# ethanhe42/epipolar-transformers

Hardware: AMD Instinct MI355X
Metric: multi-view images/sec at H36M 4-view 256x256 bs=32 (pair-views/s, whole layer forward) (higher is better)
Workload: dtype f32 (split-fp16 MFMA, f32 accumulate); 1 GPU; configs[1]: epipolarposeR head, 4 views x 32 frames = 128 pairs/GPU, C=256, 64x64, K=64, z+BN+residual, eval; partition=frames, layout=NHWC (channels_last), pairs_per_gpu=128, variant=0, launch=kernel by kernel from Python

## Files before the change

epipolar_transformers_amd/_lib.py:

```python
from __future__ import annotations

import ctypes
import os

_PKG = os.path.dirname(os.path.abspath(__file__))
LIB_PATH = os.environ.get("EPIPOLAR_AMD_LIB") or os.path.join(_PKG, "lib", "libepipolar_amd.so")

ET_CAM_STRIDE = 27
ET_VARIANT_SAFE_REDUCE = 1
ET_VARIANT_NO_TAP_CACHE = 2
ET_VARIANT_PIXEL_INTERLEAVE = 4
ET_VARIANT_BATCH4 = 8
ET_VARIANT_OCC5 = 16
ET_VARIANT_OCC6 = 32
ET_VARIANT_BASELINE = 256
ET_VARIANT_PIPELINE = 512
ET_VARIANT_MULTI2 = 1024
ET_VARIANT_MULTI4 = 2048
ET_VARIANT_BWD_ATOMIC = 4096
ET_VARIANT_BWD_UNSORTED = 8192
ET_VARIANT_NO_TILE = 16384
ET_VARIANT_TILE_SPLIT = 32768
ET_VARIANT_TILE_CLASSIC = 65536
ET_VARIANT_WS_SETPRIO = 262144
ET_VARIANT_TILE_EXACT = 524288
ET_VARIANT_WS_BAND = 1048576
ET_VARIANT_BWD_SPLIT_IN_PLACE = 2097152
ET_ABI_VERSION = 13
ET_GENERAL_POOLING = 1
ET_GENERAL_PRIOR_MUL = 2
ET_GENERAL_COSINE = 4
ET_GENERAL_ATTENTION_MAX = 8
ET_GENERAL_SIM_PRIOR = 16


class EpipolarAmdError(RuntimeError):
    pass


class EtLayerDesc(ctypes.Structure):

    _fields_ = [
        ("N", ctypes.c_int32), ("C", ctypes.c_int32), ("H", ctypes.c_int32), ("W", ctypes.c_int32),
        ("K", ctypes.c_int32),
        ("xmin", ctypes.c_float), ("ymin", ctypes.c_float), ("xmax", ctypes.c_float), ("ymax", ctypes.c_float),
        ("eps", ctypes.c_float), ("downsample", ctypes.c_float),
        ("image_resize", ctypes.c_float), ("predict_resize", ctypes.c_float),
        ("correct_normalize", ctypes.c_int32), ("align_corners", ctypes.c_int32),
        ("softmax_scale", ctypes.c_float), ("softmax_enabled", ctypes.c_int32),
        ("src_grad_mask", ctypes.c_int32), ("variant", ctypes.c_int32),
    ]


_P = ctypes.c_void_p
_D = ctypes.POINTER(EtLayerDesc)
_SIGNATURES = {
    "et_abi_version": (ctypes.c_int, []),
    "et_last_error": (ctypes.c_char_p, []),
    "et_sample_locs": (ctypes.c_int, [_D, _P, _P, _P, _P, _P, _P]),
    "et_epipolar_forward": (ctypes.c_int, [_D, _P, _P, _P, _P, _P, _P, _P, _P, _P, _P, _P, _P]),
    "et_epipolar_forward_general": (ctypes.c_int, [_D] + [_P] * 8 + [ctypes.c_int32] * 3 + [_P] * 4),
    "et_epipolar_backward_general": (ctypes.c_int, [_D] + [_P] * 9 + [ctypes.c_int32] * 3 + [_P] * 5),
    "et_epipolar_forward_workspace_bytes": (ctypes.c_size_t, [_D]),
    "et_epipolar_forward_workspace_stats_offset": (ctypes.c_size_t, [_D]),
    "et_epipolar_forward_workspace_error_offset": (ctypes.c_size_t, [_D]),
    "et_epipolar_forward_tiled": (ctypes.c_int, [_D] + [_P] * 12 + [ctypes.c_size_t, _P]),
    "et_epipolar_forward_fused": (ctypes.c_int, [_D] + [_P] * 12 + [ctypes.c_int32, _P, ctypes.c_size_t, _P]),
    "et_epipolar_backward_tiled_workspace_bytes": (ctypes.c_size_t, [_D]),
    "et_epipolar_backward_tiled": (ctypes.c_int, [_D, _P, _P, _P, _P, _P, _P, _P, _P, _P, _P, ctypes.c_size_t, _P]),
    "et_epipolar_backward_tiled_attn": (ctypes.c_int, [_D, _P, _P, _P, _P, _P, _P, _P, _P, _P, _P, _P, ctypes.c_size_t, _P]),
    "et_epipolar_backward_workspace_bytes": (ctypes.c_size_t, [_D]),
    "et_epipolar_backward": (ctypes.c_int, [_D, _P, _P, _P, _P, _P, _P, _P, _P, _P, _P, ctypes.c_size_t, _P]),
    "et_residual_epilogue": (ctypes.c_int, [ctypes.c_int64, ctypes.c_int32, _P, _P, _P, _P, _P, _P, _P, _P]),
    "et_residual_gemm_packed_bytes": (ctypes.c_size_t, []),
    "et_residual_gemm_pack": (ctypes.c_int, [_P, _P, _P]),
    "et_residual_gemm": (ctypes.c_int, [ctypes.c_int64, ctypes.c_int32, _P, _P, _P, _P, _P, _P]),
    "et_z_batch_stats_workspace_bytes": (ctypes.c_size_t, [ctypes.c_int64]),
    "et_z_batch_stats": (ctypes.c_int, [ctypes.c_int64, ctypes.c_int32, _P, _P, _P, _P, _P, _P, _P, ctypes.c_size_t, _P]),
    "et_z_wgrad_workspace_bytes": (ctypes.c_size_t, [ctypes.c_int64]),
    "et_z_wgrad": (ctypes.c_int, [ctypes.c_int64, ctypes.c_int32, _P, _P, _P, _P, _P, ctypes.c_size_t, _P]),
    "et_z_backward_workspace_bytes": (ctypes.c_size_t, [ctypes.c_int64]),
    "et_z_backward": (ctypes.c_int, [ctypes.c_int64, ctypes.c_int32, _P, _P, _P, _P, _P, _P, ctypes.c_int32, _P, _P, _P, _P, _P,
                                     ctypes.c_size_t, _P]),
    "et_heatmap_peaks": (ctypes.c_int, [ctypes.c_int64, ctypes.c_int32, ctypes.c_int32, _P, ctypes.c_float, ctypes.c_float,
                                        ctypes.c_float, ctypes.c_int32, _P, _P, _P]),
    "et_nchw_to_nhwc": (ctypes.c_int, [ctypes.c_int32] * 4 + [_P, _P, _P]),
    "et_nhwc_to_nchw": (ctypes.c_int, [ctypes.c_int32] * 4 + [_P, _P, _P]),
    "et_debug_host_sample_setup": (ctypes.c_int, [_D, _P, _P, _P, _P, ctypes.c_int32, ctypes.c_int32, _P, _P, _P]),
    "et_debug_atomic_probe": (ctypes.c_int, [_P, ctypes.c_int64, ctypes.c_int32, ctypes.c_int32, _P]),
}

_lib = None


def exported_symbols():
    return sorted(_SIGNATURES)


def load():
    global _lib
    if _lib is not None:
        return _lib
    if not os.path.exists(LIB_PATH):
        raise EpipolarAmdError(
            "HIP library %s not found. Build it with `python -m epipolar_transformers_amd.build` "
            "(hipcc, gfx950). There is no CPU fallback for this path." % LIB_PATH)
    lib = ctypes.CDLL(LIB_PATH)
    for name, (res, args) in _SIGNATURES.items():
        fn = getattr(lib, name)
        fn.restype = res
# ... 13 lines not shown
```

epipolar_transformers_amd/csrc/et_tile_host.h:

```cpp
#pragma once
#include <algorithm>
namespace {
int tile_rows_per_pixel(const EtLayerDesc *d)
{
    const int longest = d->W > d->H ? d->W : d->H;
    return (d->K < longest) ? 4 * d->K : 4 * longest;
}
int tile_rows(const EtLayerDesc *d)
{
    if (tile_rows_per_pixel(d) > kTileRowsLarge) return kTileRowsHuge;
    return (d->W > 64 || d->H > 64) ? kTileRowsLarge : kTileRowsSmall;
}
int tile_rows_cap(const EtLayerDesc *d) { return (d->variant & ET_VARIANT_TILE_SPLIT) ? 64 : tile_rows(d); }

bool tile_eligible(const EtLayerDesc *d)
{
    if (d->C != 256 || d->K > 256) return false;
    const long long hw = (long long)d->H * d->W;
    if (hw > 16384) return false;
    return tile_rows_per_pixel(d) <= tile_rows_cap(d);
}

bool tile_ws_band(const EtLayerDesc *d)
{
    const int longest = d->W > d->H ? d->W : d->H;
    if ((d->variant & ET_VARIANT_TILE_CLASSIC) || !d->softmax_enabled || d->K > 64 || d->W < 2 || longest > kWsMaxSideBand)
        return false;
    return tile_rows(d) == kTileRowsLarge || ((d->variant & ET_VARIANT_WS_BAND) && tile_rows(d) == kTileRowsSmall);
}
bool tile_ws_two_pass(const EtLayerDesc *d)
{
    const int longest = d->W > d->H ? d->W : d->H;
    return !(d->variant & ET_VARIANT_TILE_CLASSIC) && d->softmax_enabled && d->K > 64 && d->K <= 128 && d->W >= 2 && longest <= kWsMaxSideTwoPass;
}
bool tile_ws_eligible(const EtLayerDesc *d)
{
    return (!(d->variant & ET_VARIANT_TILE_CLASSIC) && d->softmax_enabled && d->K <= 64 && d->W >= 2 &&
            tile_rows(d) == kTileRowsSmall) || tile_ws_band(d);
}
struct TileWorkspace {
    int *perm, *ovf_count, *err, *ovf_list, *stats;
    float *scales;
    float4 *segs, *band, *segs_pix;
};
constexpr size_t kTileWorkspaceHeaderWords = 64;
size_t tile_workspace_words(size_t tiles, size_t pairs, size_t hw)
{
    return kTileWorkspaceHeaderWords + tiles * kTilePix + 2 * tiles + 4 * pairs + 4 + 4 * tiles * kTilePix + 4 * tiles +
           4 * pairs * hw;
}
TileWorkspace carve_tile_workspace(void *workspace, size_t tiles, size_t pairs, size_t hw)
{
    TileWorkspace w;
    w.ovf_count = reinterpret_cast<int *>((reinterpret_cast<uintptr_t>(workspace) + 255) & ~(uintptr_t)255);
    w.err = w.ovf_count + 1;
    w.perm = w.ovf_count + kTileWorkspaceHeaderWords;
    w.ovf_list = w.perm + tiles * kTilePix;
    w.stats = w.ovf_list + tiles;
    w.scales = reinterpret_cast<float *>(w.stats + tiles);
    w.segs = reinterpret_cast<float4 *>((reinterpret_cast<uintptr_t>(w.scales + 4 * pairs) + 15) & ~(uintptr_t)15);
    w.band = w.segs + tiles * kTilePix;
    w.segs_pix = w.band + tiles;
    return w;
}

int launch_tile_order(const EtLayerDesc *desc, const float *xs, const float *ys, const float *cam, const float *feat_ref,
                      const float *feat_src, const TileWorkspace &w, int tiles_per_pair, bool header, float *scales,
                      bool ws_tables, float4 *clear, size_t clear_vec4, hipStream_t st, const char *who)
{
    const int HW = desc->H * desc->W;
    const int perm_stride = tiles_per_pair * kTilePix;
    int n2 = 64;
    while (n2 < HW) n2 <<= 1;
    const size_t lds_sort = order_uses_radix(n2) ? ((tile_order_lds_bytes(n2) + 15) & ~(size_t)15) + order_radix_extra_bytes(n2)
                                                 : tile_order_lds_bytes(n2);
    const int dev = current_device();
    ET_GRANT_LDS(tile_order_kernel, lds_sort, dev);
    unsigned long long *keys = reinterpret_cast<unsigned long long *>(w.segs);
    hipLaunchKernelGGL(tile_keys_kernel, dim3((unsigned)((HW + 255) / 256) * desc->N), dim3(256), 0, st, *desc, xs, ys, cam, perm_stride,
                       keys, w.segs_pix, header ? w.ovf_count : (int *)nullptr);
    const unsigned clear_blocks = clear ? (unsigned)std::min<size_t>(2048, (clear_vec4 + 8 * 1024 - 1) / (8 * 1024)) : 0u;
    hipLaunchKernelGGL(tile_order_kernel, dim3(desc->N + clear_blocks), dim3(1024), lds_sort, st, *desc, n2, perm_stride, keys,
                       w.segs_pix, w.perm, feat_ref, feat_src, scales, ws_tables ? w.segs : (float4 *)nullptr,
                       ws_tables ? w.band : (float4 *)nullptr, clear, clear_vec4);
    return check_launch(who);
}
}
```

epipolar_transformers_amd/csrc/kernels_forward_tile.inc:

```

typedef float f32x16 __attribute__((ext_vector_type(16)));

constexpr int kTilePix = 32;
constexpr int kTileRowsSmall = 256, kTileRowsLarge = 384, kTileRowsHuge = 512;
constexpr int kTileRowsWsLarge = 288, kWsMaxSideBand = 96, kWsMaxSideTwoPass = 128;

struct TileParams {
    FwdParams f;
    const int *perm;
    int tiles_per_pair;
    int hw_words;
    int *stats;
    int rows_cap;
    const int *tile_list;
    const int *tile_count;
    const float *scales;
};

__device__ __host__ constexpr int order_key_slot(int i) { return i + (i >> 4); }
constexpr size_t tile_order_lds_bytes(int n2) { return (size_t)order_key_slot(n2) * sizeof(unsigned long long); }
__device__ __forceinline__ unsigned long long order_key(unsigned k32, int j)
{
    return (unsigned long long)__double_as_longlong((double)(((unsigned long long)k32 << 14) | (unsigned)j));
}
constexpr unsigned long long kOrderPadKey = 0x42E0000000000000ull;
__device__ __forceinline__ int order_key_pixel(unsigned long long bits)
{
    return (int)((unsigned long long)__longlong_as_double((long long)bits) & 0x3FFFull);
}
template <int S>
__device__ __forceinline__ void order_sort_round(unsigned long long *s_key, int n2, int k, int jj_top)
{
    constexpr int R = 1 << S;
    const int jlow = jj_top >> (S - 1);
    for (int t = threadIdx.x; t < (n2 >> S); t += blockDim.x) {
        const int base = ((t & ~(jlow - 1)) << S) | (t & (jlow - 1));
        const unsigned long long flip = (base & k) == 0 ? 0ull : 0x8000000000000000ull;
        double v[R];
#pragma unroll
        for (int r = 0; r < R; ++r) v[r] = __longlong_as_double((long long)(s_key[order_key_slot(base + r * jlow)] ^ flip));
#pragma unroll
        for (int st = S - 1; st >= 0; --st)
#pragma unroll
            for (int r = 0; r < R; ++r)
                if (!(r & (1 << st))) {
                    const double a = v[r], b = v[r | (1 << st)];
                    double lo, hi;
                    asm("v_min_f64 %0, %1, %2" : "=v"(lo) : "v"(a), "v"(b));
                    asm("v_max_f64 %0, %1, %2" : "=v"(hi) : "v"(a), "v"(b));
                    v[r] = lo;
                    v[r | (1 << st)] = hi;
                }
#pragma unroll
        for (int r = 0; r < R; ++r) s_key[order_key_slot(base + r * jlow)] = (unsigned long long)__double_as_longlong(v[r]) ^ flip;
    }
    __syncthreads();
}

#ifndef ET_ORDER_RADIX
#define ET_ORDER_RADIX 0
#endif
constexpr int kOrderRadixMaxKeys = 4096, kOrderRadixMinKeys = 256;
__host__ __device__ constexpr bool order_uses_radix(int n2) { return ET_ORDER_RADIX != 0 && n2 >= kOrderRadixMinKeys && n2 <= kOrderRadixMaxKeys; }
constexpr size_t order_radix_extra_bytes(int n2) { return (size_t)n2 * 8 + (size_t)256 * (n2 >> 6) * 2 + 64; }

template <int PER>
__device__ __forceinline__ void order_radix_scan(unsigned short *s_cnt, unsigned *s_wtot)
{
    const int lane = threadIdx.x & 63, wave = threadIdx.x >> 6;
    unsigned v[PER];
    if constexpr (PER == 1) {
        v[0] = s_cnt[threadIdx.x];
    } else {
        const unsigned *src = reinterpret_cast<const unsigned *>(s_cnt) + threadIdx.x * (PER / 2);
#pragma unroll
        for (int i = 0; i < PER / 2; ++i) {
            const unsigned w = src[i];
            v[2 * i] = w & 0xFFFFu;
            v[2 * i + 1] = w >> 16;
        }
    }
    unsigned sum = 0;
#pragma unroll
    for (int i = 0; i < PER; ++i) {
        const unsigned c = v[i];
        v[i] = sum;
        sum += c;
    }
    unsigned incl = sum;
#pragma unroll
    for (int m = 1; m < kWave; m <<= 1) {
        const unsigned o = __shfl_up(incl, m);
        if (lane >= m) incl += o;
    }
    if (lane == kWave - 1) s_wtot[wave] = incl;
    __syncthreads();
    unsigned base = incl - sum;
    for (int w = 0; w < wave; ++w) base += s_wtot[w];
    if constexpr (PER == 1) {
        s_cnt[threadIdx.x] = (unsigned short)(base + v[0]);
    } else {
        unsigned *dst = reinterpret_cast<unsigned *>(s_cnt) + threadIdx.x * (PER / 2);
#pragma unroll
        for (int i = 0; i < PER / 2; ++i) dst[i] = ((base + v[2 * i]) & 0xFFFFu) | ((base + v[2 * i + 1]) << 16);
    }
}

__device__ __forceinline__ void order_radix_sort(unsigned long long *s_key, int n2, int HW)
{
    const int lane = threadIdx.x & 63, wave = threadIdx.x >> 6;
    const int G = n2 >> 6;
    unsigned long long *s_b = s_key + ((order_key_slot(n2) + 1) & ~1);
    unsigned short *s_cnt = reinterpret_cast<unsigned short *>(s_b + n2);
    unsigned *s_wtot = reinterpret_cast<unsigned *>(s_cnt + 256 * G);
    constexpr int kRounds = kOrderRadixMaxKeys / 64 / 16;
    const unsigned long long lt = (1ull << lane) - 1ull;
#pragma unroll 1
    for (int pass = 0; pass < 4; ++pass) {
        const bool fwd = (pass & 1) == 0;
        for (int i = threadIdx.x; i < 128 * G; i += blockDim.x) reinterpret_cast<unsigned *>(s_cnt)[i] = 0u;
        unsigned long long key[kRounds];
        int dgt[kRounds], rank[kRounds], cnt[kRounds];
#pragma unroll
        for (int r = 0; r < kRounds; ++r) {
            const int g = wave + 16 * r;
            dgt[r] = rank[r] = cnt[r] = 0;
            key[r] = 0ull;
            if (g < G) {
                const int i = g * kWave + lane;
                unsigned long long k = fwd ? s_key[order_key_slot(i)] : s_b[i];
                if (pass == 0) {
                    k = (i < HW) ? (unsigned long long)__longlong_as_double((long long)k) : ((0xFFFFFFFFull << 14) | (unsigned)i);
                }
                key[r] = k;
                const int d8 = (int)(k >> (14 + 8 * pass)) & 255;
                unsigned long long peers = ~0ull;
#pragma unroll
                for (int b = 0; b < 8; ++b) {
                    const bool bit = (d8 >> b) & 1;
                    const unsigned long long bal = __builtin_amdgcn_ballot_w64(bit);
                    peers &= bit ? bal : ~bal;
                }
                dgt[r] = d8;
                rank[r] = __popcll(peers & lt);
                cnt[r] = __popcll(peers);
            }
        }
        __syncthreads();
#pragma unroll
        for (int r = 0; r < kRounds; ++r) {
            const int g = wave + 16 * r;
            if (g < G && rank[r] == 0) s_cnt[dgt[r] * G + g] = (unsigned short)cnt[r];
        }
        __syncthreads();
        switch (G) {
        case 64: order_radix_scan<16>(s_cnt, s_wtot); break;
        case 32: order_radix_scan<8>(s_cnt, s_wtot); break;
        case 16: order_radix_scan<4>(s_cnt, s_wtot); break;
        case 8: order_radix_scan<2>(s_cnt, s_wtot); break;
        default: order_radix_scan<1>(s_cnt, s_wtot); break;
        }
        __syncthreads();
#pragma unroll
        for (int r = 0; r < kRounds; ++r) {
            const int g = wave + 16 * r;
            if (g < G) {
                const int pos = (int)s_cnt[dgt[r] * G + g] + rank[r];
                if (pass == 3) {
                    const int pix = (int)(key[r] & 0x3FFFull);
                    s_key[order_key_slot(pos)] = (pix < HW) ? order_key((unsigned)(key[r] >> 14), pix) : kOrderPadKey;
                } else if (fwd) {
                    s_b[pos] = key[r];
                } else {
                    s_key[order_key_slot(pos)] = key[r];
                }
            }
        }
        __syncthreads();
    }
}

__global__ __launch_bounds__(256) void tile_keys_kernel(const EtLayerDesc d, const float *__restrict__ xs,
                                                        const float *__restrict__ ys, const float *__restrict__ cam_all,
                                                        int perm_stride, unsigned long long *__restrict__ keys,
                                                        float4 *__restrict__ segs_pix, int *__restrict__ zero_word)
{
    const int HW = d.H * d.W;
    const int blocks_per_pair = (HW + (int)blockDim.x - 1) / (int)blockDim.x;
    const int n = blockIdx.x / blocks_per_pair, j = (blockIdx.x - n * blocks_per_pair) * blockDim.x + threadIdx.x;
    if (zero_word && blockIdx.x == 0 && threadIdx.x < 10 && threadIdx.x != 1) zero_word[threadIdx.x] = 0;
    if (j >= HW) return;
    const float *cam = cam_all + (size_t)n * ET_CAM_STRIDE;
    const float cx = 0.5f * (d.xmin + d.xmax), cy = 0.5f * (d.ymin + d.ymax);
    const float rmax = 0.5f * sqrtf((d.xmax - d.xmin) * (d.xmax - d.xmin) + (d.ymax - d.ymin) * (d.ymax - d.ymin)) + 1.f;
    const float kPi = 3.14159265358979f;
    float th0 = atan2f(cy - cam[25], cx - cam[24]);
    if (!(fabsf(th0) <= 4.f)) th0 = 0.f;
    const int h = j / d.W, w = j - h * d.W;
    const et::Segment seg = et::epipolar_segment(d, cam, xs[w], ys[h]);
    unsigned k32 = 0xFFFFFFFFu;
    if (seg.vx != 0.f || seg.vy != 0.f) {
        float th = atan2f(seg.vy, seg.vx);
        if (th < 0.f) th += kPi;
        if (th >= kPi) th -= kPi;
        float sn, cs;
        sincosf(th, &sn, &cs);
        const float rho = (seg.sy - cy) * cs - (seg.sx - cx) * sn;
        float tk = th - th0 + 0.5f * kPi;
        tk -= kPi * floorf(tk * (1.f / kPi));
        const int tb = min(16383, max(0, (int)(tk * (16384.f / kPi))));
        const int rq = min(65535, max(0, (int)((rho / rmax * 0.5f + 0.5f) * 65535.f)));
        k32 = ((unsigned)tb << 16) | (unsigned)rq;
    }
    keys[(size_t)n * 2 * perm_stride + j] = order_key(k32, j);
    segs_pix[(size_t)n * HW + j] = make_float4(seg.sx, seg.sy, seg.vx, seg.vy);
}

__global__ __launch_bounds__(1024) void tile_order_kernel(const EtLayerDesc d, int n2, int perm_stride,
                                                          const unsigned long long *__restrict__ keys,
                                                          const float4 *__restrict__ segs_pix, int *__restrict__ perm,
                                                          const float *__restrict__ fref = nullptr,
                                                          const float *__restrict__ fsrc = nullptr,
                                                          float *__restrict__ scales = nullptr,
                                                          float4 *__restrict__ segs = nullptr,
                                                          float4 *__restrict__ band = nullptr,
                                                          float4 *__restrict__ clear = nullptr, size_t clear_vec4 = 0)
{
    extern __shared__ unsigned long long s_key[];
    if (blockIdx.x >= (unsigned)d.N) {
        const size_t nblk = gridDim.x - d.N, first = (size_t)(blockIdx.x - d.N) * blockDim.x + threadIdx.x;
        for (size_t i = first; i < clear_vec4; i += nblk * blockDim.x) clear[i] = make_float4(0.f, 0.f, 0.f, 0.f);
        return;
    }
    const int n = blockIdx.x;
    const int HW = d.H * d.W;
    const int wave = threadIdx.x >> 6, lane = threadIdx.x & 63;
    float m[2] = {0.f, 0.f};
    if (scales) {
        const int pstep = max(1, HW / 64);
        for (int which = 0; which < 2; ++which) {
            const float4 *map = reinterpret_cast<const float4 *>((which ? fsrc : fref) + (size_t)n * HW * d.C);
            for (int k = wave; k < 64; k += 16) {
                const int pix = min(k * pstep, HW - 1);
                const float4 v = map[(size_t)pix * (d.C >> 2) + (lane % (d.C >> 2))];
                m[which] = fmaxf(m[which], fmaxf(fmaxf(fabsf(v.x), fabsf(v.y)), fmaxf(fabsf(v.z), fabsf(v.w))));
            }
        }
    }
    for (int j = threadIdx.x; j < n2; j += blockDim.x)
        s_key[order_key_slot(j)] = (j < HW) ? keys[(size_t)n * 2 * perm_stride + j] : kOrderPadKey;
    __syncthreads();
    if (order_uses_radix(n2)) {
        order_radix_sort(s_key, n2, HW);
    } else {
    for (int k = 2; k <= n2; k <<= 1) {
        int jj = k >> 1;
        while (jj > 0) {
            if (jj >= 4) {
                order_sort_round<3>(s_key, n2, k, jj);
                jj >>= 3;
            } else if (jj == 2) {
                order_sort_round<2>(s_key, n2, k, jj);
                jj = 0;
            } else {
                order_sort_round<1>(s_key, n2, k, jj);
                jj = 0;
            }
        }
    }
    }
    const float4 *pair_segs = segs_pix + (size_t)n * HW;
    for (int j = threadIdx.x; j < perm_stride; j += blockDim.x) {
        const int pix = (j < HW) ? order_key_pixel(s_key[order_key_slot(j)]) : -1;
        perm[(size_t)n * perm_stride + j] = pix;
        if (segs) segs[(size_t)n * perm_stride + j] = pix >= 0 ? pair_segs[pix] : make_float4(0.f, 0.f, 0.f, 0.f);
    }
    if (band) {
        auto line_of = [&](const float4 &v, bool force, bool xm_in, float &a, float &b, bool &xm) -> bool {
            et::Segment sg;
            sg.sx = v.x; sg.sy = v.y; sg.vx = v.z; sg.vy = v.w;
            float nx0, ny0, nx1, ny1;
            et::sample_location<false>(d, sg, 0.f, et::Pow2Recips(), nx0, ny0);
            et::sample_location<false>(d, sg, 1.f, et::Pow2Recips(), nx1, ny1);
            const float x0 = et::unnormalize(nx0, d.W, d.align_corners), y0 = et::unnormalize(ny0, d.H, d.align_corners);
            const float dx = et::unnormalize(nx1, d.W, d.align_corners) - x0;
            const float dy = et::unnormalize(ny1, d.H, d.align_corners) - y0;
            xm = force ? xm_in : fabsf(dx) >= fabsf(dy);
            a = b = 0.f;
            if (xm) {
                if (dx != 0.f) b = dy / dx;
                else if (force) return false;
                a = y0 - b * x0;
            } else {
                if (dy == 0.f) return false;
                b = dx / dy;
                a = x0 - b * y0;
            }
            return fabsf(a) < 1e6f && fabsf(b) <= 4.f;
        };
        for (int t = threadIdx.x; t < perm_stride / kTilePix; t += blockDim.x) {
            const int j = t * kTilePix;
            const int pix = (j < HW) ? order_key_pixel(s_key[order_key_slot(j)]) : -1;
            float a = 0.f, b = 0.f, xmaj = 1.f;
            if (pix >= 0) {
                const float4 v = pair_segs[pix];
                bool xm = true;
                if ((v.z != 0.f || v.w != 0.f) && line_of(v, false, true, a, b, xm)) {
                    xmaj = xm ? 1.f : 0.f;
                    float4 vl = v;
                    for (int jj = min(j + kTilePix, HW) - 1; jj > j; --jj) {
                        const float4 c = pair_segs[order_key_pixel(s_key[order_key_slot(jj)])];
                        if (c.z != 0.f || c.w != 0.f) {
                            vl = c;
                            break;
                        }
                    }
                    float a2, b2;
                    bool xm2;
                    if (line_of(vl, true, xm, a2, b2, xm2)) {
                        const float ulo = -1.f, uhi = (float)(xm ? d.W : d.H);
                        const float m0 = fminf(a + b * ulo, a2 + b2 * ulo), m1 = fminf(a + b * uhi, a2 + b2 * uhi);
                        b = (m1 - m0) / (uhi - ulo);
                        a = m0 - b * ulo;
                    }
                    if (!(fabsf(a) < 1e6f)) a = 0.f, b = 0.f;
                } else {
                    a = 0.f, b = 0.f;
                }
            }
            band[(size_t)n * (perm_stride / kTilePix) + t] = make_float4(a, b, xmaj, 0.f);
        }
    }
    if (scales) {
        __syncthreads();
        float *s_red = reinterpret_cast<float *>(s_key);
        for (int which = 0; which < 2; ++which) {
            for (int o = 32; o >= 1; o >>= 1) m[which] = fmaxf(m[which], __shfl_xor(m[which], o));
            if (lane == 0) s_red[which * 16 + wave] = m[which];
        }
        __syncthreads();
        if (threadIdx.x < 2) {
            float mx = 0.f;
            for (int w = 0; w < 16; ++w) mx = fmaxf(mx, s_red[threadIdx.x * 16 + w]);
            int e = 0;
            float sc = 1.f;
            if (mx > 0.f && mx < 3e38f) {
                frexpf(mx, &e);
                e = min(60, max(-60, 11 - e));
                sc = ldexpf(1.f, e);
            }
            scales[n * 4 + threadIdx.x * 2] = sc;
            scales[n * 4 + threadIdx.x * 2 + 1] = 1.f / sc;
// ... 917 lines not shown
```

epipolar_transformers_amd/ops.py:

```python
from __future__ import annotations

import ctypes
import threading
import weakref
from dataclasses import dataclass

import numpy as np
import torch

from . import _lib
from ._lib import EtLayerDesc


@dataclass
class LayerSpec:

    H: int
    W: int
    K: int
    downsample: float = 4.0
    image_resize: float = 1.0
    predict_resize: float = 1.0
    correct_normalize: bool = True
    align_corners: bool = False
# ... 108 lines not shown
    n, h, w, cs = q.shape
    cv = map_val.shape[-1]
    if (h, w) != (spec.H, spec.W) or map_sim.shape != q.shape or map_val.shape[:3] != q.shape[:3]:
        raise ValueError("maps %s / %s / %s do not match the layer's %dx%d" %
                         (tuple(q.shape), tuple(map_sim.shape), tuple(map_val.shape), spec.H, spec.W))
    if cam.shape != (n, _lib.ET_CAM_STRIDE) or not cam.is_contiguous():
        raise ValueError("cam must be a contiguous (N,%d) tensor" % _lib.ET_CAM_STRIDE)
    if not (q.is_contiguous() and map_sim.is_contiguous() and map_val.is_contiguous()):
        raise ValueError("q / map_sim / map_val must be contiguous (N,H,W,C) tensors")
    ks = spec.K // 2 if pooling else spec.K
    if prior is not None:
        _require_gpu(prior, "prior")
        if tuple(prior.shape) != (n, ks, h, w) or not prior.is_contiguous():
            raise ValueError("prior must be (N,K',H,W) = %s, got %s" % ((n, ks, h, w), tuple(prior.shape)))
    xs, ys, steps = spec.constants(q.device)
    out = _empty((n, h, w, cv), device=q.device)
    attn = _empty((n, ks, h, w), device=q.device) if want_attn else None
    corr = _empty((n, h, w, 2), device=q.device) if want_corr else None
    flags = _general_flags(pooling, prior_mul, cosine, attention_max, sim_prior)
    d = spec.desc(n, 4)
    with torch.cuda.device(q.device):
        _lib.check(_lib.load().et_epipolar_forward_general(
            ctypes.byref(d), _ptr(xs), _ptr(ys), _ptr(steps), _ptr(cam), _ptr(q), _ptr(map_sim), _ptr(map_val),
            _ptr(prior) if prior is not None else None, cs, cv, flags, _ptr(out), _ptr(attn) if want_attn else None,
            _ptr(corr) if want_corr else None, _stream(q)), "et_epipolar_forward_general")
    return out, attn, corr


def backward_general_nhwc(spec: LayerSpec, q, map_sim, map_val, cam, grad_out, pooling=False, need_sim=True, need_val=True,
                          prior=None, prior_mul=False, cosine=False, attention_max=False, sim_prior=False, need_prior=False):
    for t, nm in ((q, "q"), (map_sim, "map_sim"), (map_val, "map_val"), (cam, "cam"), (grad_out, "grad_out")):
        _require_gpu(t, nm)
    n, h, w, cs = q.shape
    cv = map_val.shape[-1]
    if tuple(grad_out.shape) != (n, h, w, cv) or not grad_out.is_contiguous():
        raise ValueError("grad_out must be a contiguous (N,H,W,Cv) tensor")
    if not (q.is_contiguous() and map_sim.is_contiguous() and map_val.is_contiguous()):
        raise ValueError("q / map_sim / map_val must be contiguous (N,H,W,C) tensors")
    ks = spec.K // 2 if pooling else spec.K
    if prior is not None:
        _require_gpu(prior, "prior")
        if tuple(prior.shape) != (n, ks, h, w) or not prior.is_contiguous():
            raise ValueError("prior must be (N,K',H,W) = %s, got %s" % ((n, ks, h, w), tuple(prior.shape)))
    xs, ys, steps = spec.constants(q.device)
    gq = _empty(None, like=q)
    gsim = torch.zeros_like(map_sim) if need_sim else None
    gval = torch.zeros_like(map_val) if need_val else None
    gprior = _empty(None, like=prior) if (need_prior and prior is not None) else None
    d = spec.desc(n, 4)
    flags = _general_flags(pooling, prior_mul, cosine, attention_max, sim_prior)
    with torch.cuda.device(q.device):
        _lib.check(_lib.load().et_epipolar_backward_general(
            ctypes.byref(d), _ptr(xs), _ptr(ys), _ptr(steps), _ptr(cam), _ptr(q), _ptr(map_sim), _ptr(map_val),
            _ptr(prior), _ptr(grad_out), cs, cv, flags, _ptr(gq), _ptr(gsim), _ptr(gval), _ptr(gprior),
            _stream(q)), "et_epipolar_backward_general")
    return gq, gsim, gval, gprior


class GeneralAttend(torch.autograd.Function):

    @staticmethod
    def forward(ctx, q, map_sim, map_val, cam, spec: LayerSpec, pooling, prior=None, mode=None):
        mode = dict(mode or {}, pooling=bool(pooling))
        qn, m1, m2 = to_nhwc(q), to_nhwc(map_sim), to_nhwc(map_val)
        pr = None if prior is None else prior.contiguous()
        out, attn, corr = forward_general_nhwc(spec, qn, m1, m2, cam, prior=pr, **mode)
        ctx.spec, ctx.mode, ctx.has_prior = spec, mode, pr is not None
        ctx.save_for_backward(*((qn, m1, m2, cam) + ((pr,) if pr is not None else ())))
        ctx.mark_non_differentiable(attn, corr)
        return out.permute(0, 3, 1, 2), attn, corr

    @staticmethod
    def backward(ctx, grad_out, _ga, _gc):
        qn, m1, m2, cam = ctx.saved_tensors[:4]
        pr = ctx.saved_tensors[4] if ctx.has_prior else None
        gq, gs, gv, gp = backward_general_nhwc(ctx.spec, qn, m1, m2, cam, to_nhwc(grad_out), need_sim=ctx.needs_input_grad[1],
                                               need_val=ctx.needs_input_grad[2], prior=pr,
                                               need_prior=ctx.has_prior and ctx.needs_input_grad[6], **ctx.mode)
        nchw = lambda t: None if t is None else t.permute(0, 3, 1, 2)
        return nchw(gq) if ctx.needs_input_grad[0] else None, nchw(gs), nchw(gv), None, None, None, gp, None


_TILE_BITS = (_lib.ET_VARIANT_TILE_SPLIT | _lib.ET_VARIANT_TILE_CLASSIC |
              _lib.ET_VARIANT_WS_SETPRIO | _lib.ET_VARIANT_TILE_EXACT | _lib.ET_VARIANT_WS_BAND | _lib.ET_VARIANT_BWD_SPLIT_IN_PLACE)


def forward_nhwc(spec: LayerSpec, ref: torch.Tensor, src: torch.Tensor, cam: torch.Tensor,
                 want_attn=True, want_corr=True, res_bias=None, want_res_base=False, workspace=None):
    for t, nm in ((ref, "feat_ref"), (src, "feat_src"), (cam, "cam")):
        _require_gpu(t, nm)
    n, h, w, c = ref.shape
    if (h, w) != (spec.H, spec.W) or src.shape != ref.shape:
        raise ValueError("feature maps %s / %s do not match the layer's %dx%d" %
                         (tuple(ref.shape), tuple(src.shape), spec.H, spec.W))
    if cam.shape != (n, _lib.ET_CAM_STRIDE) or not cam.is_contiguous():
        raise ValueError("cam must be a contiguous (N,%d) tensor" % _lib.ET_CAM_STRIDE)
    assert ref.is_contiguous() and src.is_contiguous()
    xs, ys, steps = spec.constants(ref.device)
    out = _empty(None, like=ref)
    attn = _empty((n, spec.K, h, w), device=ref.device) if want_attn else None
    corr = _empty((n, h, w, 2), device=ref.device) if want_corr else None
    base = _empty(None, like=ref) if want_res_base else None
    if res_bias is not None:
        assert want_res_base and res_bias.is_cuda and res_bias.numel() == c and res_bias.is_contiguous()
    d = spec.desc(n, c)
    lib = _lib.load()
    ws_bytes = int(lib.et_epipolar_forward_workspace_bytes(ctypes.byref(d))) \
        if (d.variant & ~_TILE_BITS) == 0 else 0
    with torch.cuda.device(ref.device):
        if ws_bytes > 0:
            ws = workspace if workspace is not None else _workspace(ref.device, ws_bytes, "fwd")
            if ws.numel() < ws_bytes or ws.device != ref.device:
                raise ValueError("workspace of %d bytes on %s: need %d on %s" % (ws.numel(), ws.device, ws_bytes, ref.device))
            _lib.check(lib.et_epipolar_forward_tiled(ctypes.byref(d), _ptr(xs), _ptr(ys), _ptr(steps), _ptr(cam),
                                                     _ptr(ref), _ptr(src), _ptr(out), _ptr(attn), _ptr(corr),
                                                     _ptr(res_bias), _ptr(base), _ptr(ws), ctypes.c_size_t(ws_bytes),
                                                     _stream(ref)),
                       "et_epipolar_forward_tiled")
            if POISON_OUTPUTS:
                check_tile_errors(workspace=ws)
        else:
            _lib.check(lib.et_epipolar_forward(ctypes.byref(d), _ptr(xs), _ptr(ys), _ptr(steps), _ptr(cam),
                                               _ptr(ref), _ptr(src), _ptr(out), _ptr(attn), _ptr(corr),
                                               _ptr(res_bias), _ptr(base), _stream(ref)),
                       "et_epipolar_forward")
    if want_res_base:
        return out, attn, corr, base
    return out, attn, corr


def fused_layer_applies(spec: LayerSpec, c: int, n: int = 1) -> bool:
    allowed = _lib.ET_VARIANT_TILE_SPLIT | _lib.ET_VARIANT_WS_SETPRIO | _lib.ET_VARIANT_WS_BAND
    if not (c == 256 and 2 <= spec.W <= 96 and spec.H <= 96 and spec.K <= 64 and spec.softmax_enabled and
            (spec.variant & ~allowed) == 0):
        return False
    d = spec.desc(n, c)
    return int(_lib.load().et_epipolar_forward_workspace_bytes(ctypes.byref(d))) > 0


def forward_fused_nhwc(spec: LayerSpec, ref: torch.Tensor, src: torch.Tensor, cam: torch.Tensor, packed: torch.Tensor,
                       bias: torch.Tensor, want_attn=True, want_corr=True, want_out=False, workspace=None):
    for t, nm in ((ref, "feat_ref"), (src, "feat_src"), (cam, "cam"), (bias, "bias")):
        _require_gpu(t, nm)
    if not packed.is_cuda or packed.dtype != torch.uint8:
        raise TypeError("packed must be the uint8 device buffer residual_gemm_pack returns")
    n, h, w, c = ref.shape
    if (h, w) != (spec.H, spec.W) or src.shape != ref.shape or c != 256:
        raise ValueError("feature maps %s / %s do not match the layer's %dx%d x 256" % (tuple(ref.shape), tuple(src.shape), spec.H, spec.W))
    if cam.shape != (n, _lib.ET_CAM_STRIDE) or not cam.is_contiguous():
        raise ValueError("cam must be a contiguous (N,%d) tensor" % _lib.ET_CAM_STRIDE)
    need = int(_lib.load().et_residual_gemm_packed_bytes())
    if packed.numel() < need or not packed.is_contiguous() or packed.device != ref.device:
        raise ValueError("packed holds %d bytes on %s: the kernel reads %d on %s (ops.residual_gemm_pack)" %
                         (packed.numel(), packed.device, need, ref.device))
    if not (ref.is_contiguous() and src.is_contiguous()):
        raise ValueError("feat_ref / feat_src must be contiguous (N,H,W,C) tensors")
    if bias.numel() != c or not bias.is_contiguous() or bias.device != ref.device:
        raise ValueError("bias must be a contiguous float32 vector of %d values on %s" % (c, ref.device))
    if workspace is not None and (workspace.device != ref.device or workspace.dtype != torch.uint8):
        raise ValueError("workspace must be a uint8 tensor on %s" % (ref.device,))
    xs, ys, steps = spec.constants(ref.device)
    x = _empty(None, like=ref)
    out = _empty(None, like=ref) if want_out else _workspace(ref.device, ref.numel() * 4, "fwd_out_scratch").view(torch.float32)[:ref.numel()]
    attn = _empty((n, spec.K, h, w), device=ref.device) if want_attn else None
    corr = _empty((n, h, w, 2), device=ref.device) if want_corr else None
    d = spec.desc(n, c)
    lib = _lib.load()
    ws_bytes = int(lib.et_epipolar_forward_workspace_bytes(ctypes.byref(d)))
    with torch.cuda.device(ref.device):
        ws = workspace if workspace is not None else _workspace(ref.device, max(ws_bytes, 1), "fwd")
        _lib.check(lib.et_epipolar_forward_fused(ctypes.byref(d), _ptr(xs), _ptr(ys), _ptr(steps), _ptr(cam), _ptr(ref),
                                                 _ptr(src), _ptr(packed), _ptr(bias), _ptr(x), _ptr(attn), _ptr(corr),
                                                 _ptr(out), 1 if want_out else 0, _ptr(ws), ctypes.c_size_t(ws.numel()),
                                                 _stream(ref)), "et_epipolar_forward_fused")
        if POISON_OUTPUTS:
            check_tile_errors(workspace=ws)
        else:
            _poll_tile_error(ws)
    return (x, attn, corr, out) if want_out else (x, attn, corr)


_workspaces = {}
_workspaces_lock = threading.Lock()


def _prune_dead_threads_locked():
    alive = {t.ident for t in threading.enumerate()}
    for key in [k for k in _workspaces if k[4] not in alive]:
        del _workspaces[key]


def _workspace(device, nbytes: int, tag: str = "bwd") -> torch.Tensor:
    dev = torch.device(device)
    key = (dev.type, dev.index if dev.index is not None else torch.cuda.current_device(),
           torch.cuda.current_stream(dev).cuda_stream, tag, threading.get_ident())
    with _workspaces_lock:
        buf = _workspaces.get(key)
        if buf is None or buf.numel() < nbytes:
            _prune_dead_threads_locked()
            _workspaces[key] = buf = torch.zeros(nbytes, dtype=torch.uint8, device=device)
    return buf


def _own_workspace(workspace, nbytes: int, device, tag: str):
    if workspace is None:
        return _workspace(device, nbytes, tag)
    if workspace.dtype != torch.uint8 or workspace.device != device or not workspace.is_contiguous() or workspace.numel() < nbytes:
        raise ValueError("workspace must be a contiguous uint8 tensor of at least %d bytes on %s" % (nbytes, device))
    return workspace


_TILE_ERROR_OFFSET = 4


def _read_tile_error(buf: torch.Tensor) -> int:
# ... 299 lines not shown
```

include/epipolar_amd.h:

```cpp
#ifndef EPIPOLAR_AMD_H_
#define EPIPOLAR_AMD_H_

#include <stddef.h>
#include <stdint.h>

#ifdef __cplusplus
extern "C" {
#endif

#define ET_ABI_VERSION 13

typedef struct EtLayerDesc {
    int32_t N;
    int32_t C;
    int32_t H, W;
    int32_t K;
    float xmin, ymin;
    float xmax, ymax;
    float eps;
    float downsample;
    float image_resize;
    float predict_resize;
    int32_t correct_normalize;
    int32_t align_corners;
    float softmax_scale;
    int32_t softmax_enabled;
    int32_t src_grad_mask;
    int32_t variant;
} EtLayerDesc;

#define ET_CAM_STRIDE 27

#define ET_VARIANT_SAFE_REDUCE 1
#define ET_VARIANT_NO_TAP_CACHE 2
#define ET_VARIANT_PIXEL_INTERLEAVE 4
#define ET_VARIANT_BATCH4 8
#define ET_VARIANT_OCC5 16
#define ET_VARIANT_OCC6 32
#define ET_VARIANT_PIPELINE 512
#define ET_VARIANT_MULTI2 1024
#define ET_VARIANT_MULTI4 2048
#define ET_VARIANT_BWD_ATOMIC 4096
#define ET_VARIANT_BWD_UNSORTED 8192
#define ET_VARIANT_NO_TILE 16384
#define ET_VARIANT_TILE_SPLIT 32768
#define ET_VARIANT_TILE_CLASSIC 65536
#define ET_VARIANT_WS_SETPRIO 262144
#define ET_VARIANT_WS_BAND 1048576
#define ET_VARIANT_TILE_EXACT 524288
#define ET_VARIANT_BWD_SPLIT_IN_PLACE 2097152
#define ET_VARIANT_BASELINE 256
#ifdef ET_DEV_ABLATE
#define ET_VARIANT_ABLATE_NO_LOADS 64
#define ET_VARIANT_ABLATE_ONE_ROW 128
#endif

int et_abi_version(void);
const char *et_last_error(void);

int et_sample_locs(const EtLayerDesc *desc, const float *xs, const float *ys, const float *steps,
                   const float *cam, float *sample_locs, void *stream);

int et_epipolar_forward(const EtLayerDesc *desc, const float *xs, const float *ys, const float *steps,
                        const float *cam, const float *feat_ref, const float *feat_src, float *out,
                        float *attn, float *corr_pos, const float *res_bias, float *res_base,
                        void *stream);

size_t et_epipolar_forward_workspace_bytes(const EtLayerDesc *desc);
size_t et_epipolar_forward_workspace_stats_offset(const EtLayerDesc *desc);
size_t et_epipolar_forward_workspace_error_offset(const EtLayerDesc *desc);
int et_epipolar_forward_tiled(const EtLayerDesc *desc, const float *xs, const float *ys, const float *steps,
                              const float *cam, const float *feat_ref, const float *feat_src, float *out,
                              float *attn, float *corr_pos, const float *res_bias, float *res_base,
                              void *workspace, size_t workspace_bytes, void *stream);

#define ET_GENERAL_POOLING 1
#define ET_GENERAL_PRIOR_MUL 2
#define ET_GENERAL_COSINE 4
#define ET_GENERAL_ATTENTION_MAX 8
#define ET_GENERAL_SIM_PRIOR 16
int et_epipolar_forward_general(const EtLayerDesc *desc, const float *xs, const float *ys, const float *steps,
                                const float *cam, const float *q, const float *map_sim, const float *map_val,
                                const float *prior, int c_sim, int c_val, int flags, float *out, float *attn,
                                float *corr_pos, void *stream);

int et_epipolar_backward_general(const EtLayerDesc *desc, const float *xs, const float *ys, const float *steps,
                                 const float *cam, const float *q, const float *map_sim, const float *map_val,
                                 const float *prior, const float *grad_out, int c_sim, int c_val, int flags, float *grad_q,
                                 float *grad_map_sim, float *grad_map_val, float *grad_prior, void *stream);

size_t et_epipolar_backward_workspace_bytes(const EtLayerDesc *desc);
int et_epipolar_backward(const EtLayerDesc *desc, const float *xs, const float *ys, const float *steps,
                         const float *cam, const float *feat_ref, const float *feat_src,
                         const float *grad_out, float *grad_ref, float *grad_src, void *workspace,
                         size_t workspace_bytes, void *stream);

size_t et_epipolar_backward_tiled_workspace_bytes(const EtLayerDesc *desc);
int et_epipolar_backward_tiled(const EtLayerDesc *desc, const float *xs, const float *ys, const float *steps,
                               const float *cam, const float *feat_ref, const float *feat_src,
                               const float *grad_out, float *grad_ref, float *grad_src, void *workspace,
                               size_t workspace_bytes, void *stream);

int et_epipolar_backward_tiled_attn(const EtLayerDesc *desc, const float *xs, const float *ys, const float *steps,
                                    const float *cam, const float *feat_ref, const float *feat_src,
                                    const float *attn, const float *grad_out, float *grad_ref, float *grad_src,
                                    void *workspace, size_t workspace_bytes, void *stream);

int et_residual_epilogue(int64_t num_pixels, int32_t C, const float *feat, const float *out,
                         const float *y, const float *scale, const float *shift, float *finalout,
                         float *x, void *stream);

size_t et_residual_gemm_packed_bytes(void);
int et_residual_gemm_pack(const float *wf, void *packed, void *stream);
int et_residual_gemm(int64_t num_pixels, int32_t C, const float *out, const float *feat, const void *packed,
                     const float *bias, float *x, void *stream);

size_t et_z_batch_stats_workspace_bytes(int64_t num_pixels);
int et_z_batch_stats(int64_t num_pixels, int32_t C, const float *out, const void *packed_wz, const float *z_bias, float *y,
                     float *mean, float *var, void *workspace, size_t workspace_bytes, void *stream);

size_t et_z_backward_workspace_bytes(int64_t num_pixels);
int et_z_backward(int64_t num_pixels, int32_t C, const float *g, const float *y, const float *mean, const float *invstd,
                  const float *gamma, const void *packed_wzt, int32_t zresidual, float *grad_out, float *grad_y, float *grad_gamma,
                  float *grad_beta, void *workspace, size_t workspace_bytes, void *stream);

size_t et_z_wgrad_workspace_bytes(int64_t num_pixels);
int et_z_wgrad(int64_t num_pixels, int32_t C, const float *grad_y, const float *out, float *grad_w, float *grad_b, void *workspace,
               size_t workspace_bytes, void *stream);

int et_epipolar_forward_fused(const EtLayerDesc *desc, const float *xs, const float *ys, const float *steps,
                              const float *cam, const float *feat_ref, const float *feat_src, const void *packed_w,
                              const float *bias, float *x, float *attn, float *corr_pos, float *out_scratch,
                              int32_t want_out, void *workspace, size_t workspace_bytes, void *stream);
// ... 18 lines not shown
```

Measured before the change: 118,400 pair-views/s.

## Replace bitonic tile-order sort with bucket placement sort in LDS

Swaps the per-pair bitonic sorting network (and a disabled radix path) in tile_order_kernel for a bucket placement sort: keys are binned by a min/max-scaled bucket index, bucket offsets come from a block scan, and each key's rank inside its bucket is found by linear comparison. If any bucket holds more than 256 keys it falls back to the bitonic network. The aim is to cut the O(n log^2 n) compare-exchange rounds and their barriers down to a few passes. The cost is extra LDS for bucket counters, more atomics, and variable bucket sizes that depend on how the keys are distributed. The old network stays reachable through a new ORDER_NETWORK variant flag.

```diff
diff --git a/epipolar_transformers_amd/_lib.py b/epipolar_transformers_amd/_lib.py
--- a/epipolar_transformers_amd/_lib.py
+++ b/epipolar_transformers_amd/_lib.py
@@ -26,6 +26,7 @@
 ET_VARIANT_TILE_EXACT = 524288
 ET_VARIANT_WS_BAND = 1048576
 ET_VARIANT_BWD_SPLIT_IN_PLACE = 2097152
+ET_VARIANT_ORDER_NETWORK = 4194304
 ET_ABI_VERSION = 13
 ET_GENERAL_POOLING = 1
 ET_GENERAL_PRIOR_MUL = 2
diff --git a/epipolar_transformers_amd/csrc/et_tile_host.h b/epipolar_transformers_amd/csrc/et_tile_host.h
--- a/epipolar_transformers_amd/csrc/et_tile_host.h
+++ b/epipolar_transformers_amd/csrc/et_tile_host.h
@@ -72,15 +72,16 @@
     const int perm_stride = tiles_per_pair * kTilePix;
     int n2 = 64;
     while (n2 < HW) n2 <<= 1;
-    const size_t lds_sort = order_uses_radix(n2) ? ((tile_order_lds_bytes(n2) + 15) & ~(size_t)15) + order_radix_extra_bytes(n2)
-                                                 : tile_order_lds_bytes(n2);
+    const int place = (order_can_place(n2) && !(desc->variant & ET_VARIANT_ORDER_NETWORK)) ? 1 : 0;
+    const size_t lds_sort = place ? ((tile_order_lds_bytes(n2) + 15) & ~(size_t)15) + order_place_extra_bytes(n2)
+                                  : tile_order_lds_bytes(n2);
     const int dev = current_device();
     ET_GRANT_LDS(tile_order_kernel, lds_sort, dev);
     unsigned long long *keys = reinterpret_cast<unsigned long long *>(w.segs);
     hipLaunchKernelGGL(tile_keys_kernel, dim3((unsigned)((HW + 255) / 256) * desc->N), dim3(256), 0, st, *desc, xs, ys, cam, perm_stride,
                        keys, w.segs_pix, header ? w.ovf_count : (int *)nullptr);
     const unsigned clear_blocks = clear ? (unsigned)std::min<size_t>(2048, (clear_vec4 + 8 * 1024 - 1) / (8 * 1024)) : 0u;
-    hipLaunchKernelGGL(tile_order_kernel, dim3(desc->N + clear_blocks), dim3(1024), lds_sort, st, *desc, n2, perm_stride, keys,
+    hipLaunchKernelGGL(tile_order_kernel, dim3(desc->N + clear_blocks), dim3(1024), lds_sort, st, *desc, n2, perm_stride, place, keys,
                        w.segs_pix, w.perm, feat_ref, feat_src, scales, ws_tables ? w.segs : (float4 *)nullptr,
                        ws_tables ? w.band : (float4 *)nullptr, clear, clear_vec4);
     return check_launch(who);
diff --git a/epipolar_transformers_amd/csrc/kernels_forward_tile.inc b/epipolar_transformers_amd/csrc/kernels_forward_tile.inc
--- a/epipolar_transformers_amd/csrc/kernels_forward_tile.inc
+++ b/epipolar_transformers_amd/csrc/kernels_forward_tile.inc
@@ -57,127 +57,143 @@
     __syncthreads();
 }
 
-#ifndef ET_ORDER_RADIX
-#define ET_ORDER_RADIX 0
-#endif
-constexpr int kOrderRadixMaxKeys = 4096, kOrderRadixMinKeys = 256;
-__host__ __device__ constexpr bool order_uses_radix(int n2) { return ET_ORDER_RADIX != 0 && n2 >= kOrderRadixMinKeys && n2 <= kOrderRadixMaxKeys; }
-constexpr size_t order_radix_extra_bytes(int n2) { return (size_t)n2 * 8 + (size_t)256 * (n2 >> 6) * 2 + 64; }
-
-template <int PER>
-__device__ __forceinline__ void order_radix_scan(unsigned short *s_cnt, unsigned *s_wtot)
-{
-    const int lane = threadIdx.x & 63, wave = threadIdx.x >> 6;
-    unsigned v[PER];
-    if constexpr (PER == 1) {
-        v[0] = s_cnt[threadIdx.x];
-    } else {
-        const unsigned *src = reinterpret_cast<const unsigned *>(s_cnt) + threadIdx.x * (PER / 2);
-#pragma unroll
-        for (int i = 0; i < PER / 2; ++i) {
-            const unsigned w = src[i];
-            v[2 * i] = w & 0xFFFFu;
-            v[2 * i + 1] = w >> 16;
-        }
-    }
-    unsigned sum = 0;
-#pragma unroll
-    for (int i = 0; i < PER; ++i) {
-        const unsigned c = v[i];
-        v[i] = sum;
-        sum += c;
+constexpr int kOrderPlaceMaxKeys = 4096, kOrderPlaceMaxBucket = 256, kOrderPlaceSmallWords = 128;
+__host__ __device__ constexpr bool order_can_place(int n2) { return n2 <= kOrderPlaceMaxKeys; }
+__host__ __device__ constexpr int order_place_buckets(int n2) { return n2 < 1024 ? 1024 : n2; }
+constexpr size_t order_place_extra_bytes(int n2) { return (size_t)(order_place_buckets(n2) + 1 + kOrderPlaceSmallWords) * 4; }
+
+__device__ __forceinline__ bool order_placement_sort(unsigned long long *s_key, int n2, int HW,
+                                                     const unsigned long long *__restrict__ gkeys)
+{
+    constexpr int KPT = kOrderPlaceMaxKeys / 1024;
+    const int tid = threadIdx.x, lane = tid & 63, wave = tid >> 6;
+    const int NB = order_place_buckets(n2), PER = NB >> 10;
+    unsigned long long *s_tmp = s_key;
+    unsigned *s_base = reinterpret_cast<unsigned *>(s_key + ((order_key_slot(n2) + 1) & ~1));
+    unsigned *s_wlo = s_base + NB + 1, *s_whi = s_wlo + 16, *s_wtot = s_whi + 16, *s_wmax = s_wtot + 16, *s_inv = s_wmax + 16;
+    unsigned long long bits[KPT];
+    unsigned k32[KPT];
+    unsigned lo = 0xFFFFFFFFu, hi = 0u;
+#pragma unroll
+    for (int r = 0; r < KPT; ++r) {
+        const int j = tid + 1024 * r;
+        bits[r] = kOrderPadKey;
+        k32[r] = 0xFFFFFFFFu;
+        if (j < HW) {
+            bits[r] = gkeys[j];
+            k32[r] = (unsigned)((unsigned long long)__longlong_as_double((long long)bits[r]) >> 14);
+        }
+        if (k32[r] != 0xFFFFFFFFu) {
+            lo = min(lo, k32[r]);
+            hi = max(hi, k32[r]);
+        }
+    }
+    for (int i = tid; i <= NB; i += 1024) s_base[i] = 0u;
+    for (int o = 32; o >= 1; o >>= 1) {
+        lo = min(lo, (unsigned)__shfl_xor((int)lo, o));
+        hi = max(hi, (unsigned)__shfl_xor((int)hi, o));
+    }
+    if (lane == 0) s_wlo[wave] = lo, s_whi[wave] = hi;
+    __syncthreads();
+    for (int w = 0; w < 16; ++w) {
+        lo = min(lo, s_wlo[w]);
+        hi = max(hi, s_whi[w]);
+    }
+    if (lo > hi) lo = hi = 0u;
+    const float scale = (float)NB / (float)(hi - lo + 1u);
+    const unsigned long long lt = (1ull << lane) - 1ull;
+    int bucket[KPT], slot[KPT], inv_rank[KPT];
+#pragma unroll
+    for (int r = 0; r < KPT; ++r) {
+        const int j = tid + 1024 * r;
+        const bool has = k32[r] != 0xFFFFFFFFu, inv = j < HW && !has;
+        bucket[r] = slot[r] = 0;
+        if (has) {
+            bucket[r] = min(NB - 1, (int)((float)(k32[r] - lo) * scale));
+            slot[r] = (int)atomicAdd(&s_base[bucket[r]], 1u);
+        }
+        const unsigned long long bal = __builtin_amdgcn_ballot_w64(inv);
+        inv_rank[r] = __popcll(bal & lt);
+        if (lane == 0) s_inv[r * 16 + wave] = (unsigned)__popcll(bal);
+    }
+    __syncthreads();
+    unsigned c[KPT], sum = 0u, mx = 0u;
+#pragma unroll
+    for (int i = 0; i < KPT; ++i) {
+        c[i] = 0u;
+        if (i < PER) {
+            const unsigned v = s_base[tid * PER + i];
+            c[i] = sum;
+            sum += v;
+            mx = max(mx, v);
+        }
     }
     unsigned incl = sum;
-#pragma unroll
     for (int m = 1; m < kWave; m <<= 1) {
-        const unsigned o = __shfl_up(incl, m);
+        const unsigned o = (unsigned)__shfl_up((int)incl, m);
         if (lane >= m) incl += o;
     }
+    for (int o = 32; o >= 1; o >>= 1) mx = max(mx, (unsigned)__shfl_xor((int)mx, o));
     if (lane == kWave - 1) s_wtot[wave] = incl;
+    if (lane == 0) s_wmax[wave] = mx;
     __syncthreads();
-    unsigned base = incl - sum;
-    for (int w = 0; w < wave; ++w) base += s_wtot[w];
-    if constexpr (PER == 1) {
-        s_cnt[threadIdx.x] = (unsigned short)(base + v[0]);
-    } else {
-        unsigned *dst = reinterpret_cast<unsigned *>(s_cnt) + threadIdx.x * (PER / 2);
-#pragma unroll
-        for (int i = 0; i < PER / 2; ++i) dst[i] = ((base + v[2 * i]) & 0xFFFFu) | ((base + v[2 * i + 1]) << 16);
-    }
-}
-
-__device__ __forceinline__ void order_radix_sort(unsigned long long *s_key, int n2, int HW)
-{
-    const int lane = threadIdx.x & 63, wave = threadIdx.x >> 6;
-    const int G = n2 >> 6;
-    unsigned long long *s_b = s_key + ((order_key_slot(n2) + 1) & ~1);
-    unsigned short *s_cnt = reinterpret_cast<unsigned short *>(s_b + n2);
-    unsigned *s_wtot = reinterpret_cast<unsigned *>(s_cnt + 256 * G);
-    constexpr int kRounds = kOrderRadixMaxKeys / 64 / 16;
-    const unsigned long long lt = (1ull << lane) - 1ull;
-#pragma unroll 1
-    for (int pass = 0; pass < 4; ++pass) {
-        const bool fwd = (pass & 1) == 0;
-        for (int i = threadIdx.x; i < 128 * G; i += blockDim.x) reinterpret_cast<unsigned *>(s_cnt)[i] = 0u;
-        unsigned long long key[kRounds];
-        int dgt[kRounds], rank[kRounds], cnt[kRounds];
-#pragma unroll
-        for (int r = 0; r < kRounds; ++r) {
-            const int g = wave + 16 * r;
-            dgt[r] = rank[r] = cnt[r] = 0;
-            key[r] = 0ull;
-            if (g < G) {
-                const int i = g * kWave + lane;
-                unsigned long long k = fwd ? s_key[order_key_slot(i)] : s_b[i];
-                if (pass == 0) {
-                    k = (i < HW) ? (unsigned long long)__longlong_as_double((long long)k) : ((0xFFFFFFFFull << 14) | (unsigned)i);
-                }
-                key[r] = k;
-                const int d8 = (int)(k >> (14 + 8 * pass)) & 255;
-                unsigned long long peers = ~0ull;
-#pragma unroll
-                for (int b = 0; b < 8; ++b) {
-                    const bool bit = (d8 >> b) & 1;
-                    const unsigned long long bal = __builtin_amdgcn_ballot_w64(bit);
-                    peers &= bit ? bal : ~bal;
-                }
-                dgt[r] = d8;
-                rank[r] = __popcll(peers & lt);
-                cnt[r] = __popcll(peers);
-            }
+    unsigned first = incl - sum, total = 0u;
+    for (int w = 0; w < 16; ++w) {
+        const unsigned t = s_wtot[w];
+        if (w < wave) first += t;
+        total += t;
+        mx = max(mx, s_wmax[w]);
+    }
+    if (mx > (unsigned)kOrderPlaceMaxBucket) {
+#pragma unroll
+        for (int r = 0; r < KPT; ++r) {
+            const int j = tid + 1024 * r;
+            if (j < n2) s_key[order_key_slot(j)] = bits[r];
         }
         __syncthreads();
-#pragma unroll
-        for (int r = 0; r < kRounds; ++r) {
-            const int g = wave + 16 * r;
-            if (g < G && rank[r] == 0) s_cnt[dgt[r] * G + g] = (unsigned short)cnt[r];
-        }
-        __syncthreads();
-        switch (G) {
-        case 64: order_radix_scan<16>(s_cnt, s_wtot); break;
-        case 32: order_radix_scan<8>(s_cnt, s_wtot); break;
-        case 16: order_radix_scan<4>(s_cnt, s_wtot); break;
-        case 8: order_radix_scan<2>(s_cnt, s_wtot); break;
-        default: order_radix_scan<1>(s_cnt, s_wtot); break;
-        }
-        __syncthreads();
-#pragma unroll
-        for (int r = 0; r < kRounds; ++r) {
-            const int g = wave + 16 * r;
-            if (g < G) {
-                const int pos = (int)s_cnt[dgt[r] * G + g] + rank[r];
-                if (pass == 3) {
-                    const int pix = (int)(key[r] & 0x3FFFull);
-                    s_key[order_key_slot(pos)] = (pix < HW) ? order_key((unsigned)(key[r] >> 14), pix) : kOrderPadKey;
-                } else if (fwd) {
-                    s_b[pos] = key[r];
-                } else {
-                    s_key[order_key_slot(pos)] = key[r];
-                }
-            }
-        }
-        __syncthreads();
-    }
+        return false;
+    }
+#pragma unroll
+    for (int i = 0; i < KPT; ++i)
+        if (i < PER) s_base[tid * PER + i] = first + c[i];
+    if (tid == 0) s_base[NB] = total;
+    __syncthreads();
+    int b0[KPT];
+#pragma unroll
+    for (int r = 0; r < KPT; ++r) {
+        b0[r] = 0;
+        if (k32[r] != 0xFFFFFFFFu) {
+            b0[r] = (int)s_base[bucket[r]];
+            s_tmp[b0[r] + slot[r]] = bits[r];
+        }
+    }
+    __syncthreads();
+    int pos[KPT];
+#pragma unroll
+    for (int r = 0; r < KPT; ++r) {
+        const int j = tid + 1024 * r;
+        pos[r] = j;
+        if (k32[r] != 0xFFFFFFFFu) {
+            const int b1 = (int)s_base[bucket[r] + 1];
+            const int cnt = b1 - b0[r];
+            int rank = 0, i = b0[r] + (int)((unsigned)lane % (unsigned)cnt);
+            for (int t = 0; t < cnt; ++t) {
+                rank += s_tmp[i] < bits[r] ? 1 : 0;
+                if (++i == b1) i = b0[r];
+            }
+            pos[r] = b0[r] + rank;
+        } else if (j < HW) {
+            unsigned before = total + (unsigned)inv_rank[r];
+            for (int e = 0; e < r * 16 + wave; ++e) before += s_inv[e];
+            pos[r] = (int)before;
+        }
+    }
+    __syncthreads();
+#pragma unroll
+    for (int r = 0; r < KPT; ++r)
+        if (tid + 1024 * r < n2) s_key[order_key_slot(pos[r])] = bits[r];
+    __syncthreads();
+    return true;
 }
 
 __global__ __launch_bounds__(256) void tile_keys_kernel(const EtLayerDesc d, const float *__restrict__ xs,
@@ -216,7 +232,7 @@
     segs_pix[(size_t)n * HW + j] = make_float4(seg.sx, seg.sy, seg.vx, seg.vy);
 }
 
-__global__ __launch_bounds__(1024) void tile_order_kernel(const EtLayerDesc d, int n2, int perm_stride,
+__global__ __launch_bounds__(1024) void tile_order_kernel(const EtLayerDesc d, int n2, int perm_stride, int place,
                                                           const unsigned long long *__restrict__ keys,
                                                           const float4 *__restrict__ segs_pix, int *__restrict__ perm,
                                                           const float *__restrict__ fref = nullptr,
@@ -247,27 +263,30 @@
             }
         }
     }
-    for (int j = threadIdx.x; j < n2; j += blockDim.x)
-        s_key[order_key_slot(j)] = (j < HW) ? keys[(size_t)n * 2 * perm_stride + j] : kOrderPadKey;
-    __syncthreads();
-    if (order_uses_radix(n2)) {
-        order_radix_sort(s_key, n2, HW);
+    const unsigned long long *pair_keys = keys + (size_t)n * 2 * perm_stride;
+    bool sorted = false;
+    if (place) {
+        sorted = order_placement_sort(s_key, n2, HW, pair_keys);
     } else {
-    for (int k = 2; k <= n2; k <<= 1) {
-        int jj = k >> 1;
-        while (jj > 0) {
-            if (jj >= 4) {
-                order_sort_round<3>(s_key, n2, k, jj);
-                jj >>= 3;
-            } else if (jj == 2) {
-                order_sort_round<2>(s_key, n2, k, jj);
-                jj = 0;
-            } else {
-                order_sort_round<1>(s_key, n2, k, jj);
-                jj = 0;
-            }
-        }
-    }
+        for (int j = threadIdx.x; j < n2; j += blockDim.x) s_key[order_key_slot(j)] = (j < HW) ? pair_keys[j] : kOrderPadKey;
+        __syncthreads();
+    }
+    if (!sorted) {
+        for (int k = 2; k <= n2; k <<= 1) {
+            int jj = k >> 1;
+            while (jj > 0) {
+                if (jj >= 4) {
+                    order_sort_round<3>(s_key, n2, k, jj);
+                    jj >>= 3;
+                } else if (jj == 2) {
+                    order_sort_round<2>(s_key, n2, k, jj);
+                    jj = 0;
+                } else {
+                    order_sort_round<1>(s_key, n2, k, jj);
+                    jj = 0;
+                }
+            }
+        }
     }
     const float4 *pair_segs = segs_pix + (size_t)n * HW;
     for (int j = threadIdx.x; j < perm_stride; j += blockDim.x) {
diff --git a/epipolar_transformers_amd/ops.py b/epipolar_transformers_amd/ops.py
--- a/epipolar_transformers_amd/ops.py
+++ b/epipolar_transformers_amd/ops.py
@@ -214,7 +214,8 @@
 
 
 _TILE_BITS = (_lib.ET_VARIANT_TILE_SPLIT | _lib.ET_VARIANT_TILE_CLASSIC |
-              _lib.ET_VARIANT_WS_SETPRIO | _lib.ET_VARIANT_TILE_EXACT | _lib.ET_VARIANT_WS_BAND | _lib.ET_VARIANT_BWD_SPLIT_IN_PLACE)
+              _lib.ET_VARIANT_WS_SETPRIO | _lib.ET_VARIANT_TILE_EXACT | _lib.ET_VARIANT_WS_BAND | _lib.ET_VARIANT_BWD_SPLIT_IN_PLACE |
+              _lib.ET_VARIANT_ORDER_NETWORK)
 
 
 def forward_nhwc(spec: LayerSpec, ref: torch.Tensor, src: torch.Tensor, cam: torch.Tensor,
@@ -262,7 +263,7 @@
 
 
 def fused_layer_applies(spec: LayerSpec, c: int, n: int = 1) -> bool:
-    allowed = _lib.ET_VARIANT_TILE_SPLIT | _lib.ET_VARIANT_WS_SETPRIO | _lib.ET_VARIANT_WS_BAND
+    allowed = _lib.ET_VARIANT_TILE_SPLIT | _lib.ET_VARIANT_WS_SETPRIO | _lib.ET_VARIANT_WS_BAND | _lib.ET_VARIANT_ORDER_NETWORK
     if not (c == 256 and 2 <= spec.W <= 96 and spec.H <= 96 and spec.K <= 64 and spec.softmax_enabled and
             (spec.variant & ~allowed) == 0):
         return False
diff --git a/include/epipolar_amd.h b/include/epipolar_amd.h
--- a/include/epipolar_amd.h
+++ b/include/epipolar_amd.h
@@ -49,6 +49,7 @@
 #define ET_VARIANT_WS_BAND 1048576
 #define ET_VARIANT_TILE_EXACT 524288
 #define ET_VARIANT_BWD_SPLIT_IN_PLACE 2097152
+#define ET_VARIANT_ORDER_NETWORK 4194304
 #define ET_VARIANT_BASELINE 256
 #ifdef ET_DEV_ABLATE
 #define ET_VARIANT_ABLATE_NO_LOADS 64
```

Result: slower. 115,300 pair-views/s (-2.6%).
